# a-ludi/dentist

Hardware: AMD Instinct MI355X
Metric: gap-bases closed/sec (higher is better)
Workload: dtype u8

## Files before the change

dentist_amd/_lib.py:

```python
import ctypes
import os
import weakref

import numpy as np

_HERE = os.path.dirname(os.path.abspath(__file__))


def lib_path():
    return os.environ.get("DH_DEV_LIB") or os.path.join(_HERE, "libdentist_hip.so")


class DhError(RuntimeError):
    def __init__(self, code, msg):
        super().__init__(f"libdentist_hip error {code}: {msg}")
        self.code = code


class AlignOpts(ctypes.Structure):
    _fields_ = [(n, ctypes.c_int32) for n in (
        "k", "hmin", "band_shift", "tspace", "min_len", "pen", "xdrop", "max_err_ppm", "max_cand",
        "max_la", "tcap", "strands", "skip_self", "dmax", "width", "kmer_mod", "algo")]


# ... 35 lines not shown
    "right_abpos", "ins_begin", "ins_end", "comp", "cons_len", "left_diffs", "right_diffs", "join")]
    + [("cons_off", "<i8"), ("contig_right", "<i4"), ("pad", "<i4")])

CONTIG_MAPPING_DTYPE = np.dtype([("ref_contig", "<i4"), ("ref_begin", "<i4"), ("ref_end", "<i4"), ("ref_contig_length", "<i4"),
                                 ("query_contig", "<i4"), ("duplicate", "<i4"), ("complement", "<i4"), ("alignment_error", "<f4")])
GAP_SUMMARY_DTYPE = np.dtype([(f, "<i4") for f in (
    "state", "gap_length", "lhs_map", "rhs_map", "align_status", "complement", "true_contig", "true_begin", "true_end",
    "result_begin_contig", "result_begin", "result_end_contig", "result_end", "col_begin", "col_end", "reference_length",
    "query_length", "matches", "dust_ops", "dust_matches", "none_dust_ops", "none_dust_matches")])
GAP_STATES = ("unkown", "broken", "unclosed", "partiallyClosed", "closed", "ignored")
EXACT_HIT_DTYPE = np.dtype([("query", "<i4"), ("ref", "<i4"), ("begin", "<i8"), ("end", "<i8"), ("complement", "<i4"),
                            ("pad", "<i4")])

SEED_CAND_DTYPE = np.dtype([("score", "<i4"), ("aseq", "<i4"), ("apos", "<i4"), ("bpos", "<i4")])

LA_DTYPE = np.dtype([("tlen", "<i4"), ("diffs", "<i4"), ("abpos", "<i4"), ("bbpos", "<i4"),
                     ("aepos", "<i4"), ("bepos", "<i4"), ("flags", "<u4"), ("aread", "<i4"),
                     ("bread", "<i4"), ("pad", "<i4"), ("toff", "<i8")])

SYMBOLS = [
    "dh_last_error", "dh_abi_version", "dh_ctx_create", "dh_ctx_destroy", "dh_ctx_sync",
    "dh_default_align_opts", "dh_db_create", "dh_db_destroy", "dh_db_drop_cache", "dh_db_nreads",
    "dh_db_total_bases", "dh_la_set_destroy", "dh_la_set_count", "dh_la_set_trace_len",
    "dh_la_set_records", "dh_la_set_trace", "dh_la_set_tspace", "dh_get_align_stats", "dh_get_cum_stats", "dh_get_mjoin_counts", "dh_get_join_counts", "dh_get_tjoin_counts", "dh_get_seed_tier_counts", "dh_join_hit_capacity",
    "dh_ctx_release_scratch",
    "dh_align_db", "dh_seed_candidates",
    "dh_las_write", "dh_las_read", "dh_default_process_opts", "dh_collect_spanning", "dh_pileups_destroy",
    "dh_pileups_count", "dh_pileups_get", "dh_process_pileups", "dh_insertions_destroy",
    "dh_insertions_count", "dh_insertions_records", "dh_insertions_bases", "dh_insertions_bases_len",
    "dh_get_process_stats", "dh_dazz_create_dam", "dh_dazz_create_db", "dh_dazz_split", "dh_dazz_open",
    "dh_dazz_close", "dh_dazz_nreads", "dh_dazz_first_id", "dh_dazz_bases", "dh_dazz_offsets",
    "dh_dazz_origin", "dh_dazz_fpulse", "dh_dazz_header", "dh_dazz_read_mask", "dh_dazz_write_mask",
    "dh_db_set_mask", "dh_output_fasta", "dh_tile_qv", "dh_consensus", "dh_las_merge",
    "dh_collect_candidates", "dh_pileups_create", "dh_pileups_select", "dh_align_db_block", "dh_la_set_merge",
    "dh_crop_pileups", "dh_cropped_create", "dh_cropped_destroy", "dh_cropped_npiles", "dh_cropped_records",
    "dh_cropped_nreads", "dh_cropped_pile", "dh_cropped_entry", "dh_cropped_read_id", "dh_cropped_offsets",
    "dh_cropped_bases", "dh_process_cropped", "dh_translate_trace_point", "dh_db_dust", "dh_db_get_mask",
    "dh_dazz_write_track", "dh_dazz_read_track", "dh_dazz_remove", "dh_dazz_flags",
    "dh_pileupdb_write", "dh_pileupdb_read", "dh_insertiondb_write", "dh_insertiondb_read", "dh_insertiondb_merge", "dh_chaindb_destroy",
    "dh_chaindb_npiles", "dh_chaindb_pile_counts", "dh_chaindb_nread_alignments", "dh_chaindb_read_alignment_counts",
    "dh_chaindb_nseeded", "dh_chaindb_seeded", "dh_chaindb_nlas", "dh_chaindb_las", "dh_chaindb_ntrace",
    "dh_chaindb_trace", "dh_chaindb_ninsertions", "dh_chaindb_insertions", "dh_chaindb_bases", "dh_chaindb_read_ids",
    "dh_insertions_write_db", "dh_pileups_write_db", "dh_pileups_flat", "dh_collect_filter",
    "dh_map_reads", "dh_validate_regions", "dh_propagate_mask", "dh_db_mask_coverage", "dh_max_coverage_reads", "dh_max_improper_coverage_reads",
    "dh_default_scaffold_opts", "dh_scaffold_pileups", "dh_scaffold_npiles", "dh_scaffold_nentries", "dh_scaffold_joins",
    "dh_scaffold_entries", "dh_scaffold_destroy", "dh_scaffold_spanning", "dh_scaffold_gap_pileups", "dh_cropped_create2",
    "dh_cropped_kind", "dh_get_process_work", "dh_scaffold_pileups_cb", "dh_scaffold_pileups_resolved", "dh_comm_unique_id", "dh_comm_create", "dh_comm_create_local", "dh_comm_destroy",
# ... 348 lines not shown
        out = (ctypes.c_int64 * 2)()
        lib().dh_get_mjoin_counts.argtypes = [ctypes.c_void_p, ctypes.c_void_p, ctypes.c_int32]
        _check(lib().dh_get_mjoin_counts(self._h, out, int(reset)))
        return int(out[0]), int(out[1])

    def join_counts(self, reset=False):
        out = (ctypes.c_int64 * 4)()
        lib().dh_get_join_counts.argtypes = [ctypes.c_void_p, ctypes.c_void_p, ctypes.c_int32]
        _check(lib().dh_get_join_counts(self._h, out, int(reset)))
        return tuple(int(x) for x in out)

    def tjoin_counts(self, reset=False):
        out = (ctypes.c_int64 * 4)()
        lib().dh_get_tjoin_counts.argtypes = [ctypes.c_void_p, ctypes.c_void_p, ctypes.c_int32]
        _check(lib().dh_get_tjoin_counts(self._h, out, int(reset)))
        return tuple(int(x) for x in out)

    def seed_tier_counts(self, reset=False):
        out = (ctypes.c_int64 * 2)()
        lib().dh_get_seed_tier_counts.argtypes = [ctypes.c_void_p, ctypes.c_void_p, ctypes.c_int32]
        _check(lib().dh_get_seed_tier_counts(self._h, out, int(reset)))
        return int(out[0]), int(out[1])

    def cum_stats(self, reset=False):
        st = CumStats()
        _check(lib().dh_get_cum_stats(self._h, ctypes.byref(st), int(reset)))
        return st

    def remap_skipping_reads(self, contigs, reads, contig_ids, read_ids, opts, allowance):
        ci = np.ascontiguousarray(contig_ids, dtype=np.int32)
        ri = np.ascontiguousarray(read_ids, dtype=np.int32)
        h = ctypes.c_void_p()
        L = lib()
        L.dh_remap_skipping_reads.argtypes = [ctypes.c_void_p, ctypes.c_void_p, ctypes.c_void_p, ctypes.c_void_p, ctypes.c_int32,
                                              ctypes.c_void_p, ctypes.c_int32, ctypes.c_void_p, ctypes.c_int32,
                                              ctypes.POINTER(ctypes.c_void_p)]
        _check(L.dh_remap_skipping_reads(self._h, contigs._h, reads._h, ci.ctypes.data, len(ci), ri.ctypes.data, len(ri),
                                         ctypes.byref(opts), int(allowance), ctypes.byref(h)))
        las, trace, _ = _take_la_set(h)
        return las, trace

    def align_db_transposed(self, A, B, opts, select_best=False):
        h, h2 = ctypes.c_void_p(), ctypes.c_void_p()
        _check(lib().dh_align_db_transposed(self._h, A._h, B._h, ctypes.byref(opts), int(select_best), ctypes.byref(h),
                                            ctypes.byref(h2)))
        las, trace, _ = _take_la_set(h)
# ... 1882 lines not shown
```

dentist_amd/csrc/dh_api.cpp:

```cpp
#include <cstring>

#include "dh_internal.h"

static_assert(sizeof(dh_align_opts) == sizeof(DhOpts), "opts layout");
static_assert(sizeof(dh_la) == sizeof(DhLa), "la layout");
static_assert(sizeof(dh_la) == 48, "la size");

static thread_local std::string g_err;

int dh_fail(int code, const std::string &msg)
{
    g_err = msg;
    return code;
}
#define fail dh_fail

extern "C" const char *dh_last_error(void) { return g_err.c_str(); }
extern "C" int32_t dh_abi_version(void) { return 4; }



extern "C" int dh_ctx_create(int32_t device, void *stream, dh_ctx **out)
{
    if (!out) return fail(DH_EINVAL, "dh_ctx_create: out is NULL");
// ... 116 lines not shown
    return DH_OK;
}

extern "C" int dh_get_tjoin_counts(dh_ctx *c, int64_t *out4, int32_t reset)
{
    if (!c || !out4) return fail(DH_EINVAL, "dh_get_tjoin_counts: NULL");
    out4[0] = c->tj_calls;
    out4[1] = c->tj_fallbacks;
    out4[2] = c->tj_last_hits;
    out4[3] = c->tj_reruns;
    if (reset) c->tj_calls = c->tj_fallbacks = c->tj_last_hits = c->tj_reruns = 0;
    return DH_OK;
}

extern "C" int dh_get_seed_tier_counts(dh_ctx *c, int64_t *out2, int32_t reset)
{
    if (!c || !out2) return fail(DH_EINVAL, "dh_get_seed_tier_counts: NULL");
    out2[0] = c->seed_mid_chunks;
    out2[1] = c->seed_mid_redone;
    if (reset) c->seed_mid_chunks = c->seed_mid_redone = 0;
    return DH_OK;
}

extern "C" int dh_get_join_counts(dh_ctx *c, int64_t *out4, int32_t reset)
{
    if (!c || !out4) return fail(DH_EINVAL, "dh_get_join_counts: NULL");
    out4[0] = c->join_launches;
    out4[1] = c->join_reruns;
    out4[2] = c->join_last_hits;
    out4[3] = c->join_first_cap;
    if (reset) c->join_launches = c->join_reruns = c->join_last_hits = c->join_first_cap = 0;
    return DH_OK;
}

extern "C" int dh_get_align_stats(dh_ctx *c, dh_align_stats *out)
{
    if (!c || !out) return fail(DH_EINVAL, "dh_get_align_stats: NULL");
    *out = c->stats;
    return DH_OK;
}

extern "C" int dh_get_cum_stats(dh_ctx *c, dh_cum_stats *out, int32_t reset)
{
    if (!c || !out) return fail(DH_EINVAL, "dh_get_cum_stats: NULL");
    *out = c->cum;
    if (reset) c->cum = dh_cum_stats();
// ... 24 lines not shown
```

dentist_amd/csrc/dh_seed.hip:

```cpp
#include <hip/hip_runtime.h>
#include <type_traits>
#include <algorithm>
#include <cstdlib>
#include <stdio.h>
#include <stdint.h>
#include <stdlib.h>

#include "dh_device.h"
#include "dh_join.h"

#define LANES 64

#include "dh_kmer.h"


__device__ int g_seed_sort_refine = 1;
#define HIT_QBITS 24
#define HIT_QMASK ((1u << HIT_QBITS) - 1u)
#define SEED_THREADS 512
#define SEED_LOOKUP_THREADS 512
#define SEED_CCAP 256

__device__ __forceinline__ int64_t hitD(uint64_t h) { return (int64_t)(h >> HIT_QBITS); }
__device__ __forceinline__ int32_t hitQ(uint64_t h) { return (int32_t)(h & HIT_QMASK); }

__device__ __forceinline__ int32_t hit_cov(const uint64_t *h, int32_t i, int32_t k)
{
    if (i > 0 && hitD(h[i - 1]) == hitD(h[i])) {
        const int32_t dq = hitQ(h[i]) - hitQ(h[i - 1]);
        return dq < k ? dq : k;
    }
    return k;
}

#ifdef DH_SEED_PROF
__device__ unsigned long long g_seed_prof[12];
__device__ __forceinline__ unsigned long long *seed_prof_lds()
{
    __shared__ unsigned long long s_prof[12];
    return s_prof;
}
#define SP(i) if (tid == 0) { const unsigned long long t_ = wall_clock64(); seed_prof_lds()[i] += t_ - tp_; tp_ = t_; }
#else
#define SP(i)
#endif
#define HIT_DBITS 39
template <int LCAP, bool JOIN, int NT, int CC>
__device__ void seed_item(const DbView &B, const IndexView &ix, const JoinView &jv,
                          const DhOpts &o, int32_t read0, int32_t work, int32_t slab,
                          DhCand *__restrict__ cand_out, int32_t *__restrict__ ncand_out,
                          int32_t *__restrict__ nhits_out, int32_t *__restrict__ status,
                          uint64_t *__restrict__ gbuf, int32_t gcap, const int32_t *__restrict__ read_list)
{
    constexpr bool RANK_ALL = LCAP > 0 && NT <= LANES && LCAP <= 8 * NT;
    constexpr bool SLIM = LCAP > 0 && LCAP <= 4096 && NT > LANES && NT < SEED_THREADS;
    constexpr bool FB_LDS = LCAP > 0 && LCAP <= 4096;
    __shared__ uint64_t lhits[LCAP > 0 ? LCAP : 1];
    __shared__ DhCand cands[2 * CC];
    __shared__ int64_t cband[2 * CC];
    __shared__ __attribute__((aligned(8))) uint32_t bsum_l[FB_LDS ? LCAP : 1];
    __shared__ __attribute__((aligned(8))) uint16_t bhead_l[FB_LDS ? LCAP : 1];
    __shared__ int32_t s_n, s_nc;

    const int32_t r = read_list ? read_list[work] : read0 + work;
    const int32_t item = 2 * r;
    uint64_t *hits = LCAP > 0 ? lhits : gbuf + (int64_t)slab * (2 * (int64_t)gcap + (gcap + 1) / 2);
    const int32_t CAP = LCAP > 0 ? LCAP : gcap;
    const int tid = threadIdx.x;
#ifdef DH_SEED_PROF
    unsigned long long tp_ = wall_clock64();
#endif
    if (tid == 0) {
        s_n = 0;
        s_nc = 0;
    }
    __syncthreads();
    const int64_t bo = B.off[r];
    const int32_t blen = (int32_t)(B.off[r + 1] - bo);
    const uint8_t *b = B.bases + bo;
// ... 583 lines not shown
            const int32_t mid = (lo + hi) >> 1;
            if (hits[mid] >> 63)
                hi = mid;
            else
                lo = mid + 1;
        }
        nhits_out[item] = lo;
        nhits_out[item + 1] = n - lo;
    }
    SP(1)
    constexpr bool FASTB = LCAP <= 8192 || (JOIN && LCAP == 16384);
    constexpr bool FB_BIG = LCAP == 0;
    constexpr bool FB_WIDE = LCAP == 0 || LCAP == 16384;
    using bsum_t = typename std::conditional<FB_WIDE, uint64_t, uint32_t>::type;
    using bhead_t = typename std::conditional<FB_WIDE, uint32_t, uint16_t>::type;
    constexpr int HSH = FB_WIDE ? 32 : 18;
    constexpr bsum_t CMASK = ((bsum_t)1 << HSH) - 1;
    bsum_t *bsum = FB_LDS ? (bsum_t *)bsum_l
                          : (FB_BIG ? (bsum_t *)(hits + gcap) : (bsum_t *)(gbuf + (int64_t)slab * gcap));
    bhead_t *bhead = FB_LDS ? (bhead_t *)bhead_l : (bhead_t *)(bsum + (LCAP > 0 ? LCAP : gcap));
    __shared__ bsum_t s_wsum[NT / LANES];
    __shared__ int32_t s_nbig;
    constexpr int NBIG = NT <= LANES ? 8 : (SLIM ? 16 : ((LCAP > 0 && LCAP <= 4096) ? 128 : 64));
    __shared__ int32_t bigc[NBIG][4];
    __shared__ unsigned long long s_bestkeys[NBIG];
    const int bs = o.band_shift;
    auto emit_cand = [&](int32_t slot, int32_t best_first, int32_t P, int64_t band) {
        const int64_t D = hitD(hits[best_first]) & ((1ll << HIT_DBITS) - 1);
        const int32_t q = hitQ(hits[best_first]);
        const int64_t gv = D - ix.sepv + q;
        const int32_t lo = ix.page_seq[gv >> 12];
        cands[slot].score = P;
        cands[slot].aseq = lo;
        cands[slot].apos = (int32_t)(gv - ix.goff[lo]);
        cands[slot].bpos = q;
        cband[slot] = band;
    };
    auto serial_seed = [&](int32_t i, int32_t e1) {
        int32_t best_first = i, best_cov = -1, run_first = i;
        for (int32_t x = i; x < e1; x++) {
            bool linked = false;
            if (x > i && hitD(hits[x]) == hitD(hits[x - 1]))
                linked = (hitQ(hits[x]) - hitQ(hits[x - 1])) <= k;
            if (!linked) run_first = x;
            const int32_t cov = k + hitQ(hits[x]) - hitQ(hits[run_first]);
            if (cov > best_cov) {
                best_cov = cov;
                best_first = run_first;
// ... 1 lines not shown
        }
        return best_first;
    };
    if (FASTB) {
        if (tid == 0) s_nbig = 0;
        const int32_t per = (n + NT - 1) / NT;
        const int32_t x0 = tid * per, x1 = min(n, x0 + per);
        bsum_t acc = 0;
        for (int32_t i = x0; i < x1; i++) {
            const bool head = i == 0 || (hitD(hits[i - 1]) >> bs) != (hitD(hits[i]) >> bs);
            acc += ((bsum_t)(head ? 1u : 0u) << HSH) | (bsum_t)hit_cov(hits, i, k);
            if (LCAP == 0) bsum[i] = acc;
        }
        bsum_t incl = acc;
        for (int off = 1; off < LANES; off <<= 1) {
            const bsum_t up = __shfl_up(incl, off, LANES);
            if ((tid & (LANES - 1)) >= off) incl += up;
        }
        if ((tid & (LANES - 1)) == LANES - 1) s_wsum[tid / LANES] = incl;
        __syncthreads();
        bsum_t base = incl - acc;
        for (int wv = 0; wv < tid / LANES; wv++) base += s_wsum[wv];
        bsum_t run = base;
        for (int32_t i = x0; i < x1; i++) {
            const bool head = i == 0 || (hitD(hits[i - 1]) >> bs) != (hitD(hits[i]) >> bs);
            bsum_t v;
            if (LCAP == 0)
                v = bsum[i] + base;
            else {
                run += ((bsum_t)(head ? 1u : 0u) << HSH) | (bsum_t)hit_cov(hits, i, k);
                v = run;
            }
            bsum[i] = v;
            if (head) bhead[(v >> HSH) - 1] = (bhead_t)i;
        }
        __syncthreads();
        SP(2)
        const int32_t nheads = (int32_t)(bsum[n - 1] >> HSH);
        auto band_cov = [&](int32_t rnk) {
            const int32_t st_ = bhead[rnk], en_ = rnk + 1 < nheads ? bhead[rnk + 1] : n;
            return (int32_t)((bsum[en_ - 1] & CMASK) - (st_ ? (bsum[st_ - 1] & CMASK) : (bsum_t)0));
        };
        for (int32_t rnk = tid; rnk < nheads; rnk += NT) {
            const int32_t i = bhead[rnk];
            const int64_t band = hitD(hits[i]) >> bs;
            int32_t covm1 = 0, cov1 = 0, cov2 = 0, e1;
            const int32_t cov0 = band_cov(rnk);
            if (rnk > 0 && (hitD(hits[bhead[rnk - 1]]) >> bs) == band - 1) covm1 = band_cov(rnk - 1);
            int32_t nx = rnk + 1;
            e1 = nx < nheads ? bhead[nx] : n;
            if (nx < nheads && (hitD(hits[bhead[nx]]) >> bs) == band + 1) {
                cov1 = band_cov(nx);
                nx++;
                e1 = nx < nheads ? bhead[nx] : n;
            }
            if (nx < nheads && (hitD(hits[bhead[nx]]) >> bs) == band + 2) cov2 = band_cov(nx);
            const int32_t P = cov0 + cov1, Pm1 = covm1 + cov0, Pp1 = cov1 + cov2;
            if (P < o.hmin || P < Pm1 || P <= Pp1) continue;
            const int32_t slot = atomicAdd(&s_nc, 1);
            if (slot >= 2 * CC) continue;
            if (e1 - i > 16) {
                const int32_t bslot = atomicAdd(&s_nbig, 1);
                if (bslot < NBIG) {
                    bigc[bslot][0] = i;
                    bigc[bslot][1] = e1;
                    bigc[bslot][2] = P;
                    bigc[bslot][3] = slot;
                    continue;
                }
            }
            emit_cand(slot, serial_seed(i, e1), P, band);
        }
        __syncthreads();
        SP(8)
        constexpr int GW = SLIM ? LANES : 16;
        const int32_t nbig = min(s_nbig, NBIG);
        const int gl = tid & (GW - 1);
        for (int32_t bc = tid / GW; bc < nbig; bc += NT / GW) {
            const int32_t i = bigc[bc][0], e1 = bigc[bc][1];
            unsigned long long best = 0ull;
            int32_t carry = i;
            for (int32_t base = i; base < e1; base += GW) {
                const int32_t x = base + gl;
                const bool valid = x < e1;
                const uint64_t h = valid ? hits[x] : 0ull;
                const uint64_t hp = valid && x > i ? hits[x - 1] : 0ull;
                const uint64_t hn = x + 1 < e1 ? hits[x + 1] : 0ull;
                const bool linked = valid && x > i && hitD(h) == hitD(hp) && (hitQ(h) - hitQ(hp)) <= k;
                int32_t f = valid && !linked ? x : -1;
                for (int off = 1; off < GW; off <<= 1) {
                    const int32_t up = __shfl_up(f, off, GW);
                    if (gl >= off) f = up > f ? up : f;
                }
                f = carry > f ? carry : f;
                carry = __shfl(f, GW - 1, GW);
                const bool last = valid && (x + 1 >= e1 || hitD(hn) != hitD(h) || (hitQ(hn) - hitQ(h)) > k);
                if (last) {
                    const uint32_t cov = (uint32_t)(k + hitQ(h) - hitQ(hits[f]));
                    const unsigned long long key = ((unsigned long long)cov << 32) | (uint32_t)(0x7FFFFFFF - f);
                    best = key > best ? key : best;
                }
            }
            for (int off = GW / 2; off > 0; off >>= 1) {
                const unsigned long long ot = __shfl_xor(best, off, GW);
                best = ot > best ? ot : best;
            }
            if (gl == 0) s_bestkeys[bc] = best;
        }
        __syncthreads();
        SP(9)
        for (int32_t bc = tid; bc < nbig; bc += NT)
            emit_cand(bigc[bc][3], 0x7FFFFFFF - (int32_t)(uint32_t)s_bestkeys[bc], bigc[bc][2], hitD(hits[bigc[bc][0]]) >> bs);
    } else {
        for (int32_t i = tid; i < n; i += NT) {
            const int64_t band = hitD(hits[i]) >> bs;
            if (i > 0 && (hitD(hits[i - 1]) >> bs) == band) continue;
            int32_t covm1 = 0, cov0 = 0, cov1 = 0, cov2 = 0, e1;
            for (int32_t j = i - 1; j >= 0 && (hitD(hits[j]) >> bs) == band - 1; j--)
                covm1 += hit_cov(hits, j, k);
            int32_t j = i;
            for (; j < n && (hitD(hits[j]) >> bs) == band; j++) cov0 += hit_cov(hits, j, k);
            for (; j < n && (hitD(hits[j]) >> bs) == band + 1; j++) cov1 += hit_cov(hits, j, k);
            e1 = j;
            for (; j < n && (hitD(hits[j]) >> bs) == band + 2; j++) cov2 += hit_cov(hits, j, k);
            const int32_t P = cov0 + cov1, Pm1 = covm1 + cov0, Pp1 = cov1 + cov2;
            if (P < o.hmin || P < Pm1 || P <= Pp1) continue;
            const int32_t slot = atomicAdd(&s_nc, 1);
            if (slot < 2 * CC) emit_cand(slot, serial_seed(i, e1), P, band);
        }
    }
    __syncthreads();
    SP(3)
    int32_t nc = s_nc;
    if (nc > 2 * CC) {
        if (tid == 0) {
            ncand_out[item] = ncand_out[item + 1] = CC < SEED_CCAP ? -1 : -2;
            if (CC < SEED_CCAP) {
                nhits_out[item] = n;
                nhits_out[item + 1] = 0;
            }
        }
        return;
    }
    __shared__ int32_t crank_s[LCAP > 0 ? 1 : 2 * CC];
    int32_t *crank = LCAP > 0 ? (int32_t *)lhits : crank_s;
    __shared__ int32_t s_ncs[2];
    constexpr int BSTR = HIT_DBITS;
    auto strand_of = [&](int32_t c) { return (int32_t)((cband[c] >> (BSTR - bs)) & 1); };
    if (tid < 2) s_ncs[tid] = 0;
    __syncthreads();
    for (int32_t c = tid; c < nc; c += NT) {
        const int32_t st = strand_of(c);
        const int32_t sc = cands[c].score;
        const int64_t bc = cband[c];
        int32_t rank = 0;
#pragma unroll 4
        for (int32_t x = 0; x < nc; x++) {
            const int64_t bx = cband[x];
            const int32_t sx = cands[x].score;
            rank += ((int32_t)((bx >> (BSTR - bs)) & 1) == st && (sx > sc || (sx == sc && bx < bc))) ? 1 : 0;
        }
        crank[c] = rank;
        atomicAdd(&s_ncs[st], 1);
    }
    __syncthreads();
    for (int32_t c = tid; c < nc; c += NT) {
        const int32_t rank = crank[c], st = strand_of(c);
        if (rank >= o.max_cand) continue;
        int32_t pos = rank;
        if (o.skip_self == 2) {
            pos = 0;
            const int32_t ac = cands[c].aseq;
#pragma unroll 4
            for (int32_t x = 0; x < nc; x++) {
                const int32_t ax = cands[x].aseq, rx = crank[x];
                pos += (strand_of(x) == st && rx < o.max_cand && (ax < ac || (ax == ac && rx < rank))) ? 1 : 0;
            }
        }
        cand_out[(int64_t)(item + st) * o.max_cand + pos] = cands[c];
    }
    if (tid < 2) ncand_out[item + tid] = s_ncs[tid] < o.max_cand ? s_ncs[tid] : o.max_cand;
    SP(4)
#ifdef DH_SEED_PROF
    if (tid == 0) seed_prof_lds()[7] += 1ull;
#endif
}
template <int LCAP, bool JOIN, int NT = SEED_THREADS, int CC = SEED_CCAP>
__global__ void __launch_bounds__(NT, NT <= LANES ? 4 : (NT < SEED_THREADS ? 5 : ((LCAP > 0 && LCAP <= 2048) ? 6 : (LCAP == 16384 ? 2 : 4))))
k_seed(DbView B, IndexView ix, JoinView jv, DhOpts o, int32_t read0,
       int32_t nreads, DhCand *__restrict__ cand_out, int32_t *__restrict__ ncand_out,
       int32_t *__restrict__ nhits_out, int32_t *__restrict__ status, uint64_t *__restrict__ gbuf,
       int32_t gcap, const int32_t *__restrict__ read_list, uint32_t *__restrict__ queue)
{
    __shared__ int32_t s_work;
    constexpr int32_t BATCH = (JOIN && LCAP > 0 && LCAP <= 2048) ? 8 : 1;
#ifdef DH_SEED_PROF
    if (threadIdx.x == 0)
        for (int i = 0; i < 12; i++) seed_prof_lds()[i] = 0;
#endif
    for (;;) {
        __syncthreads();
        if (threadIdx.x == 0) s_work = (int32_t)atomicAdd(queue, (uint32_t)BATCH);
        __syncthreads();
        const int32_t work0 = s_work;
        if (work0 >= nreads) break;
#pragma unroll 1
        for (int32_t wi = 0; wi < BATCH; wi++) {
            const int32_t work = work0 + wi;
            if (work >= nreads) break;
            if (wi) __syncthreads();
            seed_item<LCAP, JOIN, NT, CC>(B, ix, jv, o, read0, work, (int32_t)blockIdx.x, cand_out, ncand_out, nhits_out,
                                          status, gbuf, gcap, read_list);
        }
    }
#ifdef DH_SEED_PROF
    if (threadIdx.x == 0)
        for (int i = 0; i < 12; i++)
            if (seed_prof_lds()[i]) atomicAdd(&g_seed_prof[i], seed_prof_lds()[i]);
#endif
}
#define SEED_INST(C, J)                                                                           \
    template __global__ void k_seed<C, J>(DbView, IndexView, JoinView, DhOpts, int32_t, int32_t,  \
                                          DhCand *, int32_t *, int32_t *, int32_t *, uint64_t *, int32_t, \
                                          const int32_t *, uint32_t *);
SEED_INST(1024, false)
SEED_INST(2048, false)
SEED_INST(4096, false)
SEED_INST(8192, false)
SEED_INST(16384, false)
SEED_INST(0, false)
SEED_INST(2048, true)
template __global__ void k_seed<512, true, 64, 32>(DbView, IndexView, JoinView, DhOpts, int32_t, int32_t, DhCand *, int32_t *, int32_t *,
                                                   int32_t *, uint64_t *, int32_t, const int32_t *, uint32_t *);
template __global__ void k_seed<2048, true, 256, 64>(DbView, IndexView, JoinView, DhOpts, int32_t, int32_t, DhCand *, int32_t *, int32_t *,
                                                     int32_t *, uint64_t *, int32_t, const int32_t *, uint32_t *);
SEED_INST(4096, true)
SEED_INST(8192, true)
SEED_INST(16384, true)
SEED_INST(0, true)


template <int C, bool J, int NT, int CC>
// ... 16 lines not shown

struct SeedLaunch {
    hipStream_t st;
    DbView B;
    IndexView ix;
    JoinView jv;
    DhOpts o;
    int32_t read0, nreads;
    DhCand *cand;
    int32_t *ncand, *nhits, *status;
    const int32_t *read_list;
    uint32_t *queue;
    int32_t ncu;
};
template <int C, bool J, int NT = SEED_THREADS, int CC = SEED_CCAP>
static void launch_seed(const SeedLaunch &a, uint64_t *gbuf, int32_t gcap)
{
    hipLaunchKernelGGL((k_seed<C, J, NT, CC>), dim3(seed_grid<C, J, NT, CC>(a.nreads, a.ncu)), dim3(NT), 0, a.st, a.B, a.ix,
                       a.jv, a.o, a.read0, a.nreads, a.cand, a.ncand, a.nhits, a.status, gbuf, gcap, a.read_list, a.queue);
}

static void seed_sort_switch()
{
    static int cur = 1;
    const int want = getenv("DH_SEED_NO_REFINE") ? 0 : 1;
    if (want != cur) {
        (void)hipDeviceSynchronize();
        (void)hipMemcpyToSymbol(HIP_SYMBOL(g_seed_sort_refine), &want, sizeof(int));
        cur = want;
    }
}

extern "C" void dhk_seed(hipStream_t st, int cap, DbView B, IndexView ix, DhOpts o,
                         int32_t item0, int32_t nitems, DhCand *cand, int32_t *ncand, int32_t *nhits,
                         int32_t *status, uint32_t *queue, int32_t ncu, uint64_t *fscr)
{
    if (nitems <= 0) return;
    seed_sort_switch();
    const SeedLaunch a = {st, B, ix, JoinView{}, o, item0 / 2, nitems / 2, cand, ncand, nhits, status, nullptr, queue, ncu};
    if (cap <= 1024)
        launch_seed<1024, false>(a, nullptr, 0);
    else if (cap <= 2048)
        launch_seed<2048, false>(a, nullptr, 0);
    else if (cap <= 4096)
        launch_seed<4096, false>(a, nullptr, 0);
    else if (cap <= 8192)
        launch_seed<8192, false>(a, fscr, DH_SEED_FSCR_WORDS);
    else
        launch_seed<16384, false>(a, nullptr, 0);
}

extern "C" void dhk_seed_big(hipStream_t st, DbView B, IndexView ix, DhOpts o,
                             const int32_t *read_list, int32_t nreads, uint64_t *gbuf, int32_t gcap, DhCand *cand,
// ... 17 lines not shown
        launch_seed<512, true, 64, 32>(a, nullptr, 0);
    else if (cap <= 2048 && mid_tier)
        launch_seed<2048, true, 256, 64>(a, nullptr, 0);
    else if (cap <= 2048)
        launch_seed<2048, true>(a, nullptr, 0);
    else if (cap <= 4096)
        launch_seed<4096, true>(a, nullptr, 0);
    else if (cap <= 8192)
        launch_seed<8192, true>(a, fscr, DH_SEED_FSCR_WORDS);
    else
        launch_seed<16384, true>(a, fscr, DH_SEED_FSCR_WORDS16);
}

extern "C" void dhk_seed_big_join(hipStream_t st, DbView B, IndexView ix, DhOpts o, JoinView jv, const int32_t *read_list,
                                  int32_t nreads, uint64_t *gbuf, int32_t gcap, DhCand *cand, int32_t *ncand,
                                  int32_t *nhits, int32_t *status, uint32_t *queue, int32_t ncu)
{
    if (nreads <= 0) return;
    const SeedLaunch a = {st, B, ix, jv, o, 0, nreads, cand, ncand, nhits, status, read_list, queue, ncu};
    launch_seed<0, true>(a, gbuf, gcap);
}

#ifdef DH_SEED_PROF
extern "C" void dhk_seed_prof_dump()
{
    unsigned long long h[12];
    (void)hipMemcpyFromSymbol(h, HIP_SYMBOL(g_seed_prof), sizeof(h));
    const double per = h[7] ? 1.0 / 100.0 / (double)h[7] : 0.0;
    fprintf(stderr, "[seed prof] reads %llu: fill %.1f sort %.1f (buckets %.1f scatter %.1f ranks %.1f) bcov %.1f bands %.1f (heads %.1f long ranges %.1f emit %.1f) rank %.1f us/read; %llu reads through the network\n",
            h[7], h[0] * per, (h[5] + h[6] + h[1]) * per, h[5] * per, h[6] * per, h[1] * per, h[2] * per, (h[8] + h[9] + h[3]) * per,
            h[8] * per, h[9] * per, h[3] * per, h[4] * per, h[10]);
    unsigned long long z[12] = {0};
    (void)hipMemcpyToSymbol(HIP_SYMBOL(g_seed_prof), z, sizeof(z));
}
#endif

extern "C" __global__ void __launch_bounds__(256)
k_seed_summary(const int32_t *__restrict__ ncand, const int32_t *__restrict__ nhits, int32_t n, unsigned long long *__restrict__ out)
{
    unsigned long long h = 0, c = 0, big = 0, gave = 0;
    for (int32_t i = blockIdx.x * blockDim.x + threadIdx.x; i < n; i += gridDim.x * blockDim.x) {
        const int32_t nc = ncand[i];
        h += (unsigned long long)max(nhits[i], 0);
        c += (unsigned long long)max(nc, 0);
        big += nc == -1 ? 1ull : 0ull;
        gave += nc == -2 ? 1ull : 0ull;
    }
    for (int off = 32; off > 0; off >>= 1) {
        h += __shfl_xor(h, off, 64);
        c += __shfl_xor(c, off, 64);
        big += __shfl_xor(big, off, 64);
        gave += __shfl_xor(gave, off, 64);
    }
    __shared__ unsigned long long s_part[4][4];
    if ((threadIdx.x & 63) == 0) {
        s_part[threadIdx.x >> 6][0] = h;
// ... 18 lines not shown
```

include/dentist_hip.h:

```cpp
#ifndef DENTIST_HIP_H
#define DENTIST_HIP_H

#include <stddef.h>
#include <stdint.h>

#ifdef __cplusplus
extern "C" {
#endif

#define DH_OK 0
#define DH_EINVAL (-1)
#define DH_ENODEV (-2)
#define DH_EHIP (-3)
#define DH_EOVERFLOW (-4)
#define DH_EIO (-5)
#define DH_ENOMEM (-6)

const char *dh_last_error(void);
int32_t dh_abi_version(void);

typedef struct dh_ctx dh_ctx;
int dh_ctx_create(int32_t device, void *stream, dh_ctx **out);
void dh_ctx_destroy(dh_ctx *ctx);
int dh_ctx_sync(dh_ctx *ctx);
// ... 51 lines not shown
const uint16_t *dh_la_set_trace(const dh_la_set *s);
int32_t dh_la_set_tspace(const dh_la_set *s);

typedef struct {
    int64_t hits, cands, alignments, wave_cells, las;
    int64_t b_bases;
    float ms_index, ms_seed, ms_wave, ms_gather, ms_total;
    int32_t wave_launches;
    int32_t overflow_items;
    int64_t big_items;
} dh_align_stats;
int dh_get_align_stats(dh_ctx *ctx, dh_align_stats *out);

typedef struct {
    double ms_index, ms_seed, ms_wave, ms_gather;
    int64_t wave_launches, wave_cells, alignments, las, aligned_bp, trace_values, hits, b_bases;
} dh_cum_stats;
int dh_get_cum_stats(dh_ctx *ctx, dh_cum_stats *out, int32_t reset);
int dh_ctx_release_scratch(dh_ctx *ctx);
int dh_get_mjoin_counts(dh_ctx *ctx, int64_t *out2, int32_t reset);
int dh_get_join_counts(dh_ctx *ctx, int64_t *out4, int32_t reset);
int dh_get_tjoin_counts(dh_ctx *ctx, int64_t *out4, int32_t reset);
int dh_get_seed_tier_counts(dh_ctx *ctx, int64_t *out2, int32_t reset);
int64_t dh_join_hit_capacity(const int64_t *bases, const int32_t *reads, int32_t ngroups, int32_t skip_self, double rate,
                             int64_t free_bytes);

int dh_align_db(dh_ctx *ctx, dh_db *A, dh_db *B, const dh_align_opts *opts, int32_t select_best,
                dh_la_set **out);
typedef struct { int32_t score, aseq, apos, bpos; } dh_seed_cand;
int dh_seed_candidates(dh_ctx *ctx, dh_db *A, dh_db *B, const dh_align_opts *opts,
                       dh_seed_cand *cand, int32_t *ncand, int32_t *nhits);
void dh_set_near_best(int32_t ppm);
int dh_ctx_set_near_best(dh_ctx *ctx, int32_t ppm);

int dh_align_db_block(dh_ctx *ctx, dh_db *A, dh_db *B, int32_t first, int32_t count,
                      const dh_align_opts *opts, int32_t select_best, dh_la_set **out);
int dh_align_db_transposed(dh_ctx *ctx, dh_db *A, dh_db *B, const dh_align_opts *opts, int32_t want_best,
                           dh_la_set **out, dh_la_set **out_transposed);
int dh_la_set_merge(const dh_la_set *const *sets, int32_t nsets, dh_la_set **out);

int dh_las_write(const char *path, const dh_la *las, int64_t n, const uint16_t *trace,
                 int32_t tspace);
int dh_las_read(const char *path, dh_la_set **out);
int dh_las_merge(const char *const *paths, int32_t npaths, const char *out_path);


// ... 560 lines not shown
```

Measured before the change: 2.500 million.

## Use compact band-head table and cooperative candidate ranking in large join seed tiers

For the 8192/16384-entry join seed tiers, band heads are written into a compact table placed after the hits in shared memory, so per-band coverage comes from one pair of entries instead of bhead/bsum lookups. Long bands are tracked through a slot list in the candidate array rather than a fixed-size bigc array, which removes the NBIG cap. Candidate ranking and skip-self positioning are split across groups of lanes with shuffle reductions instead of one thread per candidate. It adds an environment switch to fall back to the old layout and device counters that record which path each read took, at the cost of more code and more shared-memory use.

```diff
diff --git a/dentist_amd/_lib.py b/dentist_amd/_lib.py
--- a/dentist_amd/_lib.py
+++ b/dentist_amd/_lib.py
@@ -81,7 +81,7 @@
     "dh_last_error", "dh_abi_version", "dh_ctx_create", "dh_ctx_destroy", "dh_ctx_sync",
     "dh_default_align_opts", "dh_db_create", "dh_db_destroy", "dh_db_drop_cache", "dh_db_nreads",
     "dh_db_total_bases", "dh_la_set_destroy", "dh_la_set_count", "dh_la_set_trace_len",
-    "dh_la_set_records", "dh_la_set_trace", "dh_la_set_tspace", "dh_get_align_stats", "dh_get_cum_stats", "dh_get_mjoin_counts", "dh_get_join_counts", "dh_get_tjoin_counts", "dh_get_seed_tier_counts", "dh_join_hit_capacity",
+    "dh_la_set_records", "dh_la_set_trace", "dh_la_set_tspace", "dh_get_align_stats", "dh_get_cum_stats", "dh_get_mjoin_counts", "dh_get_join_counts", "dh_get_tjoin_counts", "dh_get_seed_tier_counts", "dh_get_seed_band_counts", "dh_join_hit_capacity",
     "dh_ctx_release_scratch",
     "dh_align_db", "dh_seed_candidates",
     "dh_las_write", "dh_las_read", "dh_default_process_opts", "dh_collect_spanning", "dh_pileups_destroy",
@@ -476,6 +476,12 @@
         _check(lib().dh_get_seed_tier_counts(self._h, out, int(reset)))
         return int(out[0]), int(out[1])
 
+    def seed_band_counts(self, reset=False):
+        out = (ctypes.c_int64 * 2)()
+        lib().dh_get_seed_band_counts.argtypes = [ctypes.c_void_p, ctypes.c_void_p, ctypes.c_int32]
+        _check(lib().dh_get_seed_band_counts(self._h, out, int(reset)))
+        return int(out[0]), int(out[1])
+
     def cum_stats(self, reset=False):
         st = CumStats()
         _check(lib().dh_get_cum_stats(self._h, ctypes.byref(st), int(reset)))
diff --git a/dentist_amd/csrc/dh_api.cpp b/dentist_amd/csrc/dh_api.cpp
--- a/dentist_amd/csrc/dh_api.cpp
+++ b/dentist_amd/csrc/dh_api.cpp
@@ -162,6 +162,19 @@
     return DH_OK;
 }
 
+extern "C" int dhk_seed_band_counts(unsigned long long *out, int reset);
+
+extern "C" int dh_get_seed_band_counts(dh_ctx *c, int64_t *out2, int32_t reset)
+{
+    if (!c || !out2) return fail(DH_EINVAL, "dh_get_seed_band_counts: NULL");
+    HIPCHK(hipSetDevice(c->device));
+    unsigned long long v[2] = {0, 0};
+    if (dhk_seed_band_counts(v, reset)) return fail(DH_EHIP, "dh_get_seed_band_counts: the counters could not be read");
+    out2[0] = (int64_t)v[0];
+    out2[1] = (int64_t)v[1];
+    return DH_OK;
+}
+
 extern "C" int dh_get_join_counts(dh_ctx *c, int64_t *out4, int32_t reset)
 {
     if (!c || !out4) return fail(DH_EINVAL, "dh_get_join_counts: NULL");
diff --git a/dentist_amd/csrc/dh_seed.hip b/dentist_amd/csrc/dh_seed.hip
--- a/dentist_amd/csrc/dh_seed.hip
+++ b/dentist_amd/csrc/dh_seed.hip
@@ -15,6 +15,13 @@
 
 
 __device__ int g_seed_sort_refine = 1;
+__device__ int g_seed_slab_bands = 0;
+__device__ unsigned long long g_seed_band_reads[2];
+__device__ __forceinline__ uint32_t *seed_band_lds()
+{
+    __shared__ uint32_t s_band_reads[2];
+    return s_band_reads;
+}
 #define HIT_QBITS 24
 #define HIT_QMASK ((1u << HIT_QBITS) - 1u)
 #define SEED_THREADS 512
@@ -34,7 +41,8 @@
 }
 
 #ifdef DH_SEED_PROF
-__device__ unsigned long long g_seed_prof[12];
+__device__ unsigned long long g_seed_prof_all[3][12];
+#define g_seed_prof g_seed_prof_all[LCAP == 8192 ? 1 : (LCAP == 16384 ? 2 : 0)]
 __device__ __forceinline__ unsigned long long *seed_prof_lds()
 {
     __shared__ unsigned long long s_prof[12];
@@ -55,6 +63,7 @@
     constexpr bool RANK_ALL = LCAP > 0 && NT <= LANES && LCAP <= 8 * NT;
     constexpr bool SLIM = LCAP > 0 && LCAP <= 4096 && NT > LANES && NT < SEED_THREADS;
     constexpr bool FB_LDS = LCAP > 0 && LCAP <= 4096;
+    constexpr bool HTAB = JOIN && NT == SEED_THREADS && (LCAP == 8192 || LCAP == 16384);
     __shared__ uint64_t lhits[LCAP > 0 ? LCAP : 1];
     __shared__ DhCand cands[2 * CC];
     __shared__ int64_t cband[2 * CC];
@@ -684,8 +693,10 @@
     __shared__ bsum_t s_wsum[NT / LANES];
     __shared__ int32_t s_nbig;
     constexpr int NBIG = NT <= LANES ? 8 : (SLIM ? 16 : ((LCAP > 0 && LCAP <= 4096) ? 128 : 64));
-    __shared__ int32_t bigc[NBIG][4];
-    __shared__ unsigned long long s_bestkeys[NBIG];
+    __shared__ int32_t bigc[HTAB ? 1 : NBIG][4];
+    __shared__ unsigned long long s_bestkeys[HTAB ? 1 : NBIG];
+    __shared__ uint16_t biglist[HTAB ? 2 * CC : 1];
+    static_assert(2 * CC <= 65536, "a candidate slot fits a biglist entry");
     const int bs = o.band_shift;
     auto emit_cand = [&](int32_t slot, int32_t best_first, int32_t P, int64_t band) {
         const int64_t D = hitD(hits[best_first]) & ((1ll << HIT_DBITS) - 1);
@@ -733,6 +744,28 @@
         bsum_t base = incl - acc;
         for (int wv = 0; wv < tid / LANES; wv++) base += s_wsum[wv];
         bsum_t run = base;
+        constexpr int TPW = (int)(sizeof(uint64_t) / sizeof(bsum_t));
+        bsum_t *htab = (bsum_t *)(hits + n);
+        bool use_tab = false;
+        int32_t nheads_tab = 0;
+        if constexpr (HTAB) {
+            static_assert(HTAB ? sizeof(bsum_t) * 8 - HSH >= (LCAP == 8192 ? 14 : 15) : true, "a position <= LCAP - 1 (and n) fits an entry");
+            bsum_t tot = 0;
+            for (int wv = 0; wv < NT / LANES; wv++) tot += s_wsum[wv];
+            nheads_tab = (int32_t)(tot >> HSH);
+            use_tab = !g_seed_slab_bands && n + (nheads_tab + 1 + TPW - 1) / TPW <= LCAP;
+            if (tid == 0) {
+                seed_band_lds()[use_tab ? 0 : 1]++;
+                if (use_tab) htab[nheads_tab] = ((bsum_t)n << HSH) | (tot & CMASK);
+            }
+        }
+        if (HTAB && use_tab) {
+            for (int32_t i = x0; i < x1; i++) {
+                const bool head = i == 0 || (hitD(hits[i - 1]) >> bs) != (hitD(hits[i]) >> bs);
+                if (head) htab[(int32_t)(run >> HSH)] = ((bsum_t)i << HSH) | (run & CMASK);
+                run += ((bsum_t)(head ? 1u : 0u) << HSH) | (bsum_t)hit_cov(hits, i, k);
+            }
+        } else
         for (int32_t i = x0; i < x1; i++) {
             const bool head = i == 0 || (hitD(hits[i - 1]) >> bs) != (hitD(hits[i]) >> bs);
             bsum_t v;
@@ -747,48 +780,94 @@
         }
         __syncthreads();
         SP(2)
-        const int32_t nheads = (int32_t)(bsum[n - 1] >> HSH);
-        auto band_cov = [&](int32_t rnk) {
-            const int32_t st_ = bhead[rnk], en_ = rnk + 1 < nheads ? bhead[rnk + 1] : n;
-            return (int32_t)((bsum[en_ - 1] & CMASK) - (st_ ? (bsum[st_ - 1] & CMASK) : (bsum_t)0));
-        };
-        for (int32_t rnk = tid; rnk < nheads; rnk += NT) {
-            const int32_t i = bhead[rnk];
-            const int64_t band = hitD(hits[i]) >> bs;
-            int32_t covm1 = 0, cov1 = 0, cov2 = 0, e1;
-            const int32_t cov0 = band_cov(rnk);
-            if (rnk > 0 && (hitD(hits[bhead[rnk - 1]]) >> bs) == band - 1) covm1 = band_cov(rnk - 1);
-            int32_t nx = rnk + 1;
-            e1 = nx < nheads ? bhead[nx] : n;
-            if (nx < nheads && (hitD(hits[bhead[nx]]) >> bs) == band + 1) {
-                cov1 = band_cov(nx);
-                nx++;
+        if constexpr (HTAB) {
+            auto head_loop = [&](const int32_t nheads, auto hpos, auto band_cov) {
+                for (int32_t rnk = tid; rnk < nheads; rnk += NT) {
+                    const int32_t i = hpos(rnk);
+                    const int64_t band = hitD(hits[i]) >> bs;
+                    int32_t covm1 = 0, cov1 = 0, cov2 = 0, e1;
+                    const int32_t cov0 = band_cov(rnk);
+                    if (rnk > 0 && (hitD(hits[hpos(rnk - 1)]) >> bs) == band - 1) covm1 = band_cov(rnk - 1);
+                    int32_t nx = rnk + 1;
+                    e1 = nx < nheads ? hpos(nx) : n;
+                    if (nx < nheads && (hitD(hits[hpos(nx)]) >> bs) == band + 1) {
+                        cov1 = band_cov(nx);
+                        nx++;
+                        e1 = nx < nheads ? hpos(nx) : n;
+                    }
+                    if (nx < nheads && (hitD(hits[hpos(nx)]) >> bs) == band + 2) cov2 = band_cov(nx);
+                    const int32_t P = cov0 + cov1, Pm1 = covm1 + cov0, Pp1 = cov1 + cov2;
+                    if (P < o.hmin || P < Pm1 || P <= Pp1) continue;
+                    const int32_t slot = atomicAdd(&s_nc, 1);
+                    if (slot >= 2 * CC) continue;
+                    if (e1 - i > 16) {
+                        const int32_t bslot = atomicAdd(&s_nbig, 1);
+                        cands[slot].score = P;
+                        cands[slot].aseq = i;
+                        cands[slot].apos = e1;
+                        biglist[bslot] = (uint16_t)slot;
+                        continue;
+                    }
+                    emit_cand(slot, serial_seed(i, e1), P, band);
+                }
+            };
+            if (use_tab) {
+                head_loop(
+                    nheads_tab, [&](int32_t rnk) { return (int32_t)(htab[rnk] >> HSH); },
+                    [&](int32_t rnk) { return (int32_t)((htab[rnk + 1] & CMASK) - (htab[rnk] & CMASK)); });
+            } else {
+                const int32_t nheads = (int32_t)(bsum[n - 1] >> HSH);
+                head_loop(
+                    nheads, [&](int32_t rnk) { return (int32_t)bhead[rnk]; },
+                    [&](int32_t rnk) {
+                        const int32_t st_ = bhead[rnk], en_ = rnk + 1 < nheads ? bhead[rnk + 1] : n;
+                        return (int32_t)((bsum[en_ - 1] & CMASK) - (st_ ? (bsum[st_ - 1] & CMASK) : (bsum_t)0));
+                    });
+            }
+        } else {
+            const int32_t nheads = (int32_t)(bsum[n - 1] >> HSH);
+            auto band_cov = [&](int32_t rnk) {
+                const int32_t st_ = bhead[rnk], en_ = rnk + 1 < nheads ? bhead[rnk + 1] : n;
+                return (int32_t)((bsum[en_ - 1] & CMASK) - (st_ ? (bsum[st_ - 1] & CMASK) : (bsum_t)0));
+            };
+            for (int32_t rnk = tid; rnk < nheads; rnk += NT) {
+                const int32_t i = bhead[rnk];
+                const int64_t band = hitD(hits[i]) >> bs;
+                int32_t covm1 = 0, cov1 = 0, cov2 = 0, e1;
+                const int32_t cov0 = band_cov(rnk);
+                if (rnk > 0 && (hitD(hits[bhead[rnk - 1]]) >> bs) == band - 1) covm1 = band_cov(rnk - 1);
+                int32_t nx = rnk + 1;
                 e1 = nx < nheads ? bhead[nx] : n;
-            }
-            if (nx < nheads && (hitD(hits[bhead[nx]]) >> bs) == band + 2) cov2 = band_cov(nx);
-            const int32_t P = cov0 + cov1, Pm1 = covm1 + cov0, Pp1 = cov1 + cov2;
-            if (P < o.hmin || P < Pm1 || P <= Pp1) continue;
-            const int32_t slot = atomicAdd(&s_nc, 1);
-            if (slot >= 2 * CC) continue;
-            if (e1 - i > 16) {
-                const int32_t bslot = atomicAdd(&s_nbig, 1);
-                if (bslot < NBIG) {
-                    bigc[bslot][0] = i;
-                    bigc[bslot][1] = e1;
-                    bigc[bslot][2] = P;
-                    bigc[bslot][3] = slot;
-                    continue;
-                }
-            }
-            emit_cand(slot, serial_seed(i, e1), P, band);
+                if (nx < nheads && (hitD(hits[bhead[nx]]) >> bs) == band + 1) {
+                    cov1 = band_cov(nx);
+                    nx++;
+                    e1 = nx < nheads ? bhead[nx] : n;
+                }
+                if (nx < nheads && (hitD(hits[bhead[nx]]) >> bs) == band + 2) cov2 = band_cov(nx);
+                const int32_t P = cov0 + cov1, Pm1 = covm1 + cov0, Pp1 = cov1 + cov2;
+                if (P < o.hmin || P < Pm1 || P <= Pp1) continue;
+                const int32_t slot = atomicAdd(&s_nc, 1);
+                if (slot >= 2 * CC) continue;
+                if (e1 - i > 16) {
+                    const int32_t bslot = atomicAdd(&s_nbig, 1);
+                    if (bslot < NBIG) {
+                        bigc[bslot][0] = i;
+                        bigc[bslot][1] = e1;
+                        bigc[bslot][2] = P;
+                        bigc[bslot][3] = slot;
+                        continue;
+                    }
+                }
+                emit_cand(slot, serial_seed(i, e1), P, band);
+            }
         }
         __syncthreads();
         SP(8)
         constexpr int GW = SLIM ? LANES : 16;
-        const int32_t nbig = min(s_nbig, NBIG);
+        const int32_t nbig = HTAB ? s_nbig : min(s_nbig, NBIG);
         const int gl = tid & (GW - 1);
         for (int32_t bc = tid / GW; bc < nbig; bc += NT / GW) {
-            const int32_t i = bigc[bc][0], e1 = bigc[bc][1];
+            const int32_t i = HTAB ? cands[biglist[bc]].aseq : bigc[bc][0], e1 = HTAB ? cands[biglist[bc]].apos : bigc[bc][1];
             unsigned long long best = 0ull;
             int32_t carry = i;
             for (int32_t base = i; base < e1; base += GW) {
@@ -816,12 +895,23 @@
                 const unsigned long long ot = __shfl_xor(best, off, GW);
                 best = ot > best ? ot : best;
             }
-            if (gl == 0) s_bestkeys[bc] = best;
+            if (gl == 0) {
+                if constexpr (HTAB)
+                    cands[biglist[bc]].bpos = 0x7FFFFFFF - (int32_t)(uint32_t)best;
+                else
+                    s_bestkeys[bc] = best;
+            }
         }
         __syncthreads();
         SP(9)
-        for (int32_t bc = tid; bc < nbig; bc += NT)
-            emit_cand(bigc[bc][3], 0x7FFFFFFF - (int32_t)(uint32_t)s_bestkeys[bc], bigc[bc][2], hitD(hits[bigc[bc][0]]) >> bs);
+        for (int32_t bc = tid; bc < nbig; bc += NT) {
+            if constexpr (HTAB) {
+                const int32_t slot = biglist[bc];
+                const DhCand d = cands[slot];
+                emit_cand(slot, d.bpos, d.score, hitD(hits[d.aseq]) >> bs);
+            } else
+                emit_cand(bigc[bc][3], 0x7FFFFFFF - (int32_t)(uint32_t)s_bestkeys[bc], bigc[bc][2], hitD(hits[bigc[bc][0]]) >> bs);
+        }
     } else {
         for (int32_t i = tid; i < n; i += NT) {
             const int64_t band = hitD(hits[i]) >> bs;
@@ -860,35 +950,83 @@
     auto strand_of = [&](int32_t c) { return (int32_t)((cband[c] >> (BSTR - bs)) & 1); };
     if (tid < 2) s_ncs[tid] = 0;
     __syncthreads();
-    for (int32_t c = tid; c < nc; c += NT) {
-        const int32_t st = strand_of(c);
-        const int32_t sc = cands[c].score;
-        const int64_t bc = cband[c];
-        int32_t rank = 0;
+    if constexpr (HTAB) {
+        int G = 4;
+        while (G < LANES && nc * 2 * G <= NT) G <<= 1;
+        const int gl = tid & (G - 1);
+        for (int32_t c0 = 0; c0 < nc; c0 += NT / G) {
+            const int32_t c = c0 + tid / G;
+            const bool on = c < nc;
+            const int32_t cc = on ? c : 0;
+            const int32_t st = strand_of(cc);
+            const int32_t sc = cands[cc].score;
+            const int64_t bc = cband[cc];
+            int32_t rank = 0;
 #pragma unroll 4
-        for (int32_t x = 0; x < nc; x++) {
-            const int64_t bx = cband[x];
-            const int32_t sx = cands[x].score;
-            rank += ((int32_t)((bx >> (BSTR - bs)) & 1) == st && (sx > sc || (sx == sc && bx < bc))) ? 1 : 0;
-        }
-        crank[c] = rank;
-        atomicAdd(&s_ncs[st], 1);
-    }
-    __syncthreads();
-    for (int32_t c = tid; c < nc; c += NT) {
-        const int32_t rank = crank[c], st = strand_of(c);
-        if (rank >= o.max_cand) continue;
-        int32_t pos = rank;
-        if (o.skip_self == 2) {
-            pos = 0;
-            const int32_t ac = cands[c].aseq;
+            for (int32_t x = gl; x < nc; x += G) {
+                const int64_t bx = cband[x];
+                const int32_t sx = cands[x].score;
+                rank += ((int32_t)((bx >> (BSTR - bs)) & 1) == st && (sx > sc || (sx == sc && bx < bc))) ? 1 : 0;
+            }
+            for (int off = G >> 1; off > 0; off >>= 1) rank += __shfl_xor(rank, off, G);
+            if (on && gl == 0) {
+                crank[c] = rank;
+                atomicAdd(&s_ncs[st], 1);
+            }
+        }
+        __syncthreads();
+        for (int32_t c0 = 0; c0 < nc; c0 += NT / G) {
+            const int32_t c = c0 + tid / G;
+            const bool on = c < nc;
+            const int32_t cc = on ? c : 0;
+            const int32_t rank = crank[cc], st = strand_of(cc);
+            const bool kept = on && rank < o.max_cand;
+            int32_t pos = 0;
+            if (o.skip_self == 2) {
+                const int32_t ac = cands[cc].aseq;
+                if (kept) {
+#pragma unroll 4
+                    for (int32_t x = gl; x < nc; x += G) {
+                        const int32_t ax = cands[x].aseq, rx = crank[x];
+                        pos += (strand_of(x) == st && rx < o.max_cand && (ax < ac || (ax == ac && rx < rank))) ? 1 : 0;
+                    }
+                }
+                for (int off = G >> 1; off > 0; off >>= 1) pos += __shfl_xor(pos, off, G);
+            } else
+                pos = rank;
+            if (kept && gl == 0) cand_out[(int64_t)(item + st) * o.max_cand + pos] = cands[cc];
+        }
+    } else {
+        for (int32_t c = tid; c < nc; c += NT) {
+            const int32_t st = strand_of(c);
+            const int32_t sc = cands[c].score;
+            const int64_t bc = cband[c];
+            int32_t rank = 0;
 #pragma unroll 4
             for (int32_t x = 0; x < nc; x++) {
-                const int32_t ax = cands[x].aseq, rx = crank[x];
-                pos += (strand_of(x) == st && rx < o.max_cand && (ax < ac || (ax == ac && rx < rank))) ? 1 : 0;
-            }
-        }
-        cand_out[(int64_t)(item + st) * o.max_cand + pos] = cands[c];
+                const int64_t bx = cband[x];
+                const int32_t sx = cands[x].score;
+                rank += ((int32_t)((bx >> (BSTR - bs)) & 1) == st && (sx > sc || (sx == sc && bx < bc))) ? 1 : 0;
+            }
+            crank[c] = rank;
+            atomicAdd(&s_ncs[st], 1);
+        }
+        __syncthreads();
+        for (int32_t c = tid; c < nc; c += NT) {
+            const int32_t rank = crank[c], st = strand_of(c);
+            if (rank >= o.max_cand) continue;
+            int32_t pos = rank;
+            if (o.skip_self == 2) {
+                pos = 0;
+                const int32_t ac = cands[c].aseq;
+#pragma unroll 4
+                for (int32_t x = 0; x < nc; x++) {
+                    const int32_t ax = cands[x].aseq, rx = crank[x];
+                    pos += (strand_of(x) == st && rx < o.max_cand && (ax < ac || (ax == ac && rx < rank))) ? 1 : 0;
+                }
+            }
+            cand_out[(int64_t)(item + st) * o.max_cand + pos] = cands[c];
+        }
     }
     if (tid < 2) ncand_out[item + tid] = s_ncs[tid] < o.max_cand ? s_ncs[tid] : o.max_cand;
     SP(4)
@@ -909,6 +1047,9 @@
     if (threadIdx.x == 0)
         for (int i = 0; i < 12; i++) seed_prof_lds()[i] = 0;
 #endif
+    constexpr bool HTAB = JOIN && NT == SEED_THREADS && (LCAP == 8192 || LCAP == 16384);
+    if constexpr (HTAB)
+        if (threadIdx.x < 2) seed_band_lds()[threadIdx.x] = 0;
     for (;;) {
         __syncthreads();
         if (threadIdx.x == 0) s_work = (int32_t)atomicAdd(queue, (uint32_t)BATCH);
@@ -920,8 +1061,12 @@
             const int32_t work = work0 + wi;
             if (work >= nreads) break;
             if (wi) __syncthreads();
-            seed_item<LCAP, JOIN, NT, CC>(B, ix, jv, o, read0, work, (int32_t)blockIdx.x, cand_out, ncand_out, nhits_out,
-                                          status, gbuf, gcap, read_list);
+            if constexpr (HTAB) {
+                [[clang::always_inline]] seed_item<LCAP, JOIN, NT, CC>(B, ix, jv, o, read0, work, (int32_t)blockIdx.x, cand_out,
+                                                                       ncand_out, nhits_out, status, gbuf, gcap, read_list);
+            } else
+                seed_item<LCAP, JOIN, NT, CC>(B, ix, jv, o, read0, work, (int32_t)blockIdx.x, cand_out, ncand_out, nhits_out,
+                                              status, gbuf, gcap, read_list);
         }
     }
 #ifdef DH_SEED_PROF
@@ -929,6 +1074,8 @@
         for (int i = 0; i < 12; i++)
             if (seed_prof_lds()[i]) atomicAdd(&g_seed_prof[i], seed_prof_lds()[i]);
 #endif
+    if constexpr (HTAB)
+        if (threadIdx.x < 2 && seed_band_lds()[threadIdx.x]) atomicAdd(&g_seed_band_reads[threadIdx.x], (unsigned long long)seed_band_lds()[threadIdx.x]);
 }
 #define SEED_INST(C, J)                                                                           \
     template __global__ void k_seed<C, J>(DbView, IndexView, JoinView, DhOpts, int32_t, int32_t,  \
@@ -991,13 +1138,30 @@
 
 static void seed_sort_switch()
 {
-    static int cur = 1;
+    static int cur = 1, cur_slab = 0;
     const int want = getenv("DH_SEED_NO_REFINE") ? 0 : 1;
     if (want != cur) {
         (void)hipDeviceSynchronize();
         (void)hipMemcpyToSymbol(HIP_SYMBOL(g_seed_sort_refine), &want, sizeof(int));
         cur = want;
     }
+    const int want_slab = getenv("DH_SEED_SLAB_BANDS") ? 1 : 0;
+    if (want_slab != cur_slab) {
+        (void)hipDeviceSynchronize();
+        (void)hipMemcpyToSymbol(HIP_SYMBOL(g_seed_slab_bands), &want_slab, sizeof(int));
+        cur_slab = want_slab;
+    }
+}
+
+extern "C" int dhk_seed_band_counts(unsigned long long *out, int reset)
+{
+    if (hipDeviceSynchronize() != hipSuccess) return 1;
+    if (hipMemcpyFromSymbol(out, HIP_SYMBOL(g_seed_band_reads), 2 * sizeof(unsigned long long)) != hipSuccess) return 1;
+    if (reset) {
+        const unsigned long long z[2] = {0, 0};
+        if (hipMemcpyToSymbol(HIP_SYMBOL(g_seed_band_reads), z, sizeof(z)) != hipSuccess) return 1;
+    }
+    return 0;
 }
 
 extern "C" void dhk_seed(hipStream_t st, int cap, DbView B, IndexView ix, DhOpts o,
@@ -1061,16 +1225,22 @@
 }
 
 #ifdef DH_SEED_PROF
+#undef g_seed_prof
 extern "C" void dhk_seed_prof_dump()
 {
-    unsigned long long h[12];
-    (void)hipMemcpyFromSymbol(h, HIP_SYMBOL(g_seed_prof), sizeof(h));
-    const double per = h[7] ? 1.0 / 100.0 / (double)h[7] : 0.0;
-    fprintf(stderr, "[seed prof] reads %llu: fill %.1f sort %.1f (buckets %.1f scatter %.1f ranks %.1f) bcov %.1f bands %.1f (heads %.1f long ranges %.1f emit %.1f) rank %.1f us/read; %llu reads through the network\n",
-            h[7], h[0] * per, (h[5] + h[6] + h[1]) * per, h[5] * per, h[6] * per, h[1] * per, h[2] * per, (h[8] + h[9] + h[3]) * per,
-            h[8] * per, h[9] * per, h[3] * per, h[4] * per, h[10]);
-    unsigned long long z[12] = {0};
-    (void)hipMemcpyToSymbol(HIP_SYMBOL(g_seed_prof), z, sizeof(z));
+    unsigned long long all[3][12];
+    (void)hipMemcpyFromSymbol(all, HIP_SYMBOL(g_seed_prof_all), sizeof(all));
+    static const char *const row[3] = {"other tiers", "8192-entry tier", "16384-entry tier"};
+    for (int t = 0; t < 3; t++) {
+        const unsigned long long *h = all[t];
+        if (!h[7]) continue;
+        const double per = 1.0 / 100.0 / (double)h[7];
+        fprintf(stderr, "[seed prof] %s, reads %llu: fill %.1f sort %.1f (buckets %.1f scatter %.1f ranks %.1f) bcov %.1f bands %.1f (heads %.1f long ranges %.1f emit %.1f) rank %.1f us/read; %llu reads through the network\n",
+                row[t], h[7], h[0] * per, (h[5] + h[6] + h[1]) * per, h[5] * per, h[6] * per, h[1] * per, h[2] * per, (h[8] + h[9] + h[3]) * per,
+                h[8] * per, h[9] * per, h[3] * per, h[4] * per, h[10]);
+    }
+    unsigned long long z[3][12] = {{0}};
+    (void)hipMemcpyToSymbol(HIP_SYMBOL(g_seed_prof_all), z, sizeof(z));
 }
 #endif
 
diff --git a/include/dentist_hip.h b/include/dentist_hip.h
--- a/include/dentist_hip.h
+++ b/include/dentist_hip.h
@@ -97,6 +97,7 @@
 int dh_get_join_counts(dh_ctx *ctx, int64_t *out4, int32_t reset);
 int dh_get_tjoin_counts(dh_ctx *ctx, int64_t *out4, int32_t reset);
 int dh_get_seed_tier_counts(dh_ctx *ctx, int64_t *out2, int32_t reset);
+int dh_get_seed_band_counts(dh_ctx *ctx, int64_t *out2, int32_t reset);
 int64_t dh_join_hit_capacity(const int64_t *bases, const int32_t *reads, int32_t ngroups, int32_t skip_self, double rate,
                              int64_t free_bytes);
 
```

After: 2.541 million (median of 6 runs). +1.6%, better.
